# 2235854410/CCVPE

Hardware: AMD Instinct MI355X
Metric: query images/sec (VIGOR, 512x512 sat / 320x640 grd) (higher is better)
Workload: dtype f32; 1 GPU; vigor_samearea_fov360_b32; variant=vigor_ori_prior, batch_per_gpu=32, global_batch=32, parallelism=image-parallel x1, all_gather of 20 B/query results, schedule=two streams per GPU (aerial encoder + orientation decoder on the second)

## Files before the change

### ccvpe_amd/_lib.py

```python
from __future__ import annotations

import ctypes as C
import os

_HERE = os.path.dirname(os.path.abspath(__file__))
LIB_PATH = os.path.join(_HERE, "csrc", "libccvpe_hip.so")

OK = 0
VARIANT_ID = {"vigor": 0, "vigor_ori_prior": 1, "kitti": 2, "oxford": 3}


class Config(C.Structure):
    _fields_ = [("variant", C.c_int32), ("circular_padding", C.c_int32), ("ori_noise", C.c_float),
                ("device", C.c_int32), ("micro_batch", C.c_int32), ("reserved", C.c_int32 * 3)]


class Outputs(C.Structure):
    _fields_ = [("logits_flattened", C.c_void_p), ("heatmap", C.c_void_p), ("ori", C.c_void_p),
                ("matching_score", C.c_void_p * 6)]


class Pose(C.Structure):
    _fields_ = [("index", C.c_int32), ("prob", C.c_float), ("cos_v", C.c_float), ("sin_v", C.c_float),
                ("angle_deg", C.c_float)]
# ... 125 lines not shown
    ("ccvpe_localize_credible", C.c_int, [C.c_void_p, C.c_void_p, C.c_int32, C.c_int32, C.c_void_p, C.c_int32, C.c_void_p, C.c_int64,
                                          C.c_void_p, C.c_int32, C.c_void_p, C.c_void_p, C.c_void_p, C.c_void_p, C.c_void_p, C.c_void_p]),
    ("ccvpe_localize_credible_cached_indexed", C.c_int, [C.c_void_p, C.c_void_p, C.c_int32, C.c_int32, C.c_void_p, C.c_int32, C.c_void_p,
                                                         C.c_int32, C.c_void_p, C.c_int64, C.c_void_p, C.c_int32, C.c_void_p, C.c_void_p,
                                                         C.c_void_p, C.c_void_p, C.c_void_p, C.c_void_p]),
    ("ccvpe_preprocess",C.c_int, [C.c_void_p, C.c_int32, C.c_int32, C.c_int32, C.c_void_p, C.c_int32,
                                   C.POINTER(C.c_float * 3), C.POINTER(C.c_float * 3), C.c_void_p, C.c_void_p]),
    ("ccvpe_preprocess_resize", C.c_int, [C.c_void_p, C.c_int32, C.c_int32, C.c_int32, C.c_int32, C.c_int32, C.c_void_p, C.c_int32,
                                          C.POINTER(C.c_float * 3), C.POINTER(C.c_float * 3), C.c_void_p, C.c_void_p, C.c_void_p]),
    ("ccvpe_preprocess_affine", C.c_int, [C.c_void_p, C.c_int32, C.c_int32, C.c_int32, C.c_void_p, C.POINTER(C.c_int32), C.c_int32,
                                          C.c_int32, C.c_int32, C.c_int32, C.c_int32, C.POINTER(C.c_float * 3), C.POINTER(C.c_float * 3),
                                          C.c_void_p, C.c_void_p]),
    ("ccvpe_preprocess_window_resize", C.c_int, [C.c_void_p, C.c_int32, C.c_int32, C.c_void_p, C.c_int32, C.c_int32, C.c_int32,
                                                 C.c_int32, C.c_int32, C.POINTER(C.c_float * 3), C.POINTER(C.c_float * 3), C.c_void_p,
                                                 C.c_void_p, C.c_void_p]),
    ("ccvpe_set_debug", C.c_int, [C.c_void_p, C.c_int32]),
    ("ccvpe_set_streams", C.c_int, [C.c_void_p, C.c_int32]),
    ("ccvpe_read_tap", C.c_int, [C.c_void_p, C.c_char_p, C.c_void_p, C.c_size_t, C.POINTER(C.c_size_t),
                                 C.POINTER(C.c_int32 * 4)]),
    ("ccvpe_debug_dump_plan", C.c_int, [C.c_void_p, C.c_char_p]),
    ("ccvpe_profile_forward", C.c_int, [C.c_void_p, C.c_void_p, C.c_int32, C.c_int32, C.c_void_p, C.c_int32,
                                        C.POINTER(Outputs), C.c_void_p]),
    ("ccvpe_profile_row", C.c_int, [C.c_void_p, C.c_int32, C.c_char_p, C.c_size_t, C.POINTER(C.c_float),
                                    C.POINTER(C.c_double), C.POINTER(C.c_double)]),
    ("ccvpe_profile_row_issued", C.c_int, [C.c_void_p, C.c_int32, C.POINTER(C.c_double)]),
    ("ccvpe_op_num_tiles", C.c_int, []),
    ("ccvpe_op_tile_name", C.c_char_p, [C.c_int32]),
    ("ccvpe_op_conv2d", C.c_int, [C.c_void_p, C.c_int32, C.c_int32, C.c_int32, C.c_int32, C.c_void_p, C.c_void_p,
                                  C.c_int32, C.c_int32, C.c_int32, C.c_int32, C.c_int32, C.c_int32, C.c_int32,
                                  C.c_void_p, C.c_int32, C.POINTER(C.c_float), C.c_void_p]),
    ("ccvpe_op_conv2d_ex", C.c_int, [C.c_void_p, C.c_void_p]),
    ("ccvpe_op_level1", C.c_int, [C.c_void_p, C.c_int32, C.c_int32, C.c_int32, C.c_int32, C.c_int32, C.c_void_p, C.c_void_p,
                                  C.c_void_p, C.c_void_p, C.c_void_p, C.c_void_p, C.c_int32, C.c_int32, C.c_void_p, C.c_void_p]),
    ("ccvpe_op_pose_rows", C.c_int, [C.c_void_p, C.c_void_p, C.c_void_p, C.c_int32, C.c_void_p, C.c_void_p]),
]


IMAGENET_MEAN = (0.485, 0.456, 0.406)
IMAGENET_STD = (0.229, 0.224, 0.225)


def preprocess(img_u8_hwc, shift=None, crop_w=None, mean=IMAGENET_MEAN, std=IMAGENET_STD):
    import torch
    lib = load()
    assert img_u8_hwc.is_cuda and img_u8_hwc.dtype == torch.uint8 and img_u8_hwc.dim() == 4 and img_u8_hwc.shape[3] == 3
    img = img_u8_hwc.contiguous()
    B, H, W, _ = img.shape
    crop_w = W if crop_w is None else int(crop_w)
    out = torch.empty((B, 3, H, crop_w), dtype=torch.float32, device=img.device)
    sh = None
    if shift is not None:
        sh = torch.as_tensor(shift, dtype=torch.int32, device=img.device).contiguous()
        assert sh.numel() == B
    m = (C.c_float * 3)(*mean)
    s = (C.c_float * 3)(*std)
    stream = torch.cuda.current_stream(img.device).cuda_stream
    rc = lib.ccvpe_preprocess(C.c_void_p(img.data_ptr()), B, H, W, C.c_void_p(sh.data_ptr()) if sh is not None else None,
                              crop_w, C.byref(m), C.byref(s), C.c_void_p(out.data_ptr()), C.c_void_p(stream))
    check(rc, "ccvpe_preprocess")
    return out


def preprocess_resize(img_u8_hwc, out_hw, shift=None, crop_w=None, mean=IMAGENET_MEAN, std=IMAGENET_STD):
    import torch
    lib = load()
    assert img_u8_hwc.is_cuda and img_u8_hwc.dtype == torch.uint8 and img_u8_hwc.dim() == 4 and img_u8_hwc.shape[3] == 3
# ... 126 lines not shown
        assert resid.is_contiguous() and resid.dtype == torch.float32 and tuple(resid.shape[:3]) == (B, OH, OW)
        d.resid = resid.data_ptr(); d.resid_ld = resid.shape[3]
    assert 1 <= len(dsts) <= 3
    d.ndst = len(dsts)
    for i, (t, coff) in enumerate(dsts):
        assert t.is_cuda and t.is_contiguous() and t.dtype == torch.float32 and tuple(t.shape[:3]) == (B, OH, OW), tuple(t.shape)
        d.dst[i].ptr = t.data_ptr(); d.dst[i].ld = t.shape[3]; d.dst[i].coff = coff
    ran_tile, ran_split, runs = C.c_int32(0), C.c_int32(0), C.c_int32(-2)
    d.ran_tile, d.ran_split, d.requested_runs = C.pointer(ran_tile), C.pointer(ran_split), C.pointer(runs)
    stream = torch.cuda.current_stream(x.device).cuda_stream
    rc = lib.ccvpe_op_conv2d_ex(C.byref(d), C.c_void_p(stream))
    check(rc, "ccvpe_op_conv2d_ex")
    return [t for t, _ in dsts], lib.ccvpe_op_tile_name(ran_tile.value).decode(), ran_split.value, runs.value


def op_level1(x_nhwc, wd, bd, wa, ba, wt, bt, score=False, tile=1, max_wg=0):
    import torch
    lib = load()
    B, h, w, Cin = x_nhwc.shape
    Cout = wt.shape[0]
    x = x_nhwc.float()
    if score:
        x = torch.cat([x[..., :1], x.new_zeros((B, h, w, 7)), x[..., 1:]], dim=-1)
    x = x.contiguous()
    ws = [t.detach().float().contiguous() for t in (wd, bd, wa, ba, wt, bt)]
    out = torch.empty((B, Cout, 2 * h, 2 * w), dtype=torch.float32, device=x.device)
    stream = torch.cuda.current_stream(x.device).cuda_stream
    rc = lib.ccvpe_op_level1(C.c_void_p(x.data_ptr()), B, 2 * h, 2 * w, Cin, 1 if score else 0, *[C.c_void_p(t.data_ptr()) for t in ws],
                             Cout, tile | (max_wg << 8), C.c_void_p(out.data_ptr()), C.c_void_p(stream))
    check(rc, "ccvpe_op_level1")
    return out, rc


def op_pose_rows(handle, logits, ori):
    import torch
    lib = load()
    logits, ori = logits.detach().float().contiguous(), ori.detach().float().contiguous()
    B = logits.shape[0]
    rows = torch.empty((B, 5), dtype=torch.float32, device=logits.device)
    stream = torch.cuda.current_stream(logits.device).cuda_stream
    check(lib.ccvpe_op_pose_rows(handle, C.c_void_p(logits.data_ptr()), C.c_void_p(ori.data_ptr()), B, C.c_void_p(rows.data_ptr()),
                                 C.c_void_p(stream)), "ccvpe_op_pose_rows")
    return rows


_lib = None


def library_digest() -> str:
    override = os.environ.get("CCVPE_LIB_PATH")
    if override:
        import hashlib
        h = hashlib.sha256()
        with open(override, "rb") as fh:
            for chunk in iter(lambda: fh.read(1 << 20), b""):
                h.update(chunk)
        return h.hexdigest()
    from . import build as _build
    return _build._digest()


def load() -> C.CDLL:
    global _lib
    if _lib is not None:
        return _lib
    try:
# ... 42 lines not shown
```

### ccvpe_amd/build.py

```python
from __future__ import annotations

import hashlib
import os
import subprocess
import sys

HERE = os.path.dirname(os.path.abspath(__file__))
CSRC = os.path.join(HERE, "csrc")
LIB = os.path.join(CSRC, "libccvpe_hip.so")
STAMP = os.path.join(CSRC, ".libccvpe_hip.stamp")
SOURCES = ["ccvpe_api.hip", "ccvpe_weights.hip", "ccvpe_plan.hip", "ccvpe_tune.hip", "kernels_igemm.hip", "kernels_igemm_bf16x3.hip", "kernels_wino.hip", "kernels_wino4.hip", "kernels_wino4x.hip", "kernels_encoder.hip", "kernels_match.hip", "kernels_tail.hip", "kernels_heading.hip", "kernels_hprior.hip", "kernels_credible.hip", "kernels_track.hip", "kernels_track_affine.hip", "kernels_track_smooth.hip", "kernels_track_smooth_affine.hip", "kernels_track_link.hip", "kernels_track_viterbi.hip", "kernels_track_viterbi_affine.hip", "kernels_track_joint.hip", "kernels_track_joint_smooth.hip", "kernels_level1.hip", "kernels_level6.hip", "kernels_mbconv.hip", "kernels_preproc.hip", "kernels_warp.hip", "kernels_pw.hip", "kernels_proj.hip", "kernels_mbimg.hip"]
HEADERS = ["kernels.h", "ticket.h", "tail_shared.h", "track_blur.h", "track_maxmul.h", "track_smooth_work.h", "igemm_common.h", "ccvpe_internal.h", "kernels_level1_tile.inc", os.path.join("..", "..", "include", "ccvpe.h")]
FLAGS = ["--offload-arch=gfx950", "-O3", "-std=c++17", "-fPIC", "-ffp-contract=off", "-Wall", "-Wno-unused-function"]
EXTRA_FLAGS = {"kernels_match.hip": ["-fno-slp-vectorize"], "kernels_track.hip": ["-fno-slp-vectorize"], "kernels_track_affine.hip": ["-fno-slp-vectorize"],
               "kernels_track_smooth.hip": ["-fno-slp-vectorize"], "kernels_track_smooth_affine.hip": ["-fno-slp-vectorize"],
               "kernels_track_link.hip": ["-fno-slp-vectorize"],
               "kernels_track_viterbi.hip": ["-fno-slp-vectorize"], "kernels_track_viterbi_affine.hip": ["-fno-slp-vectorize"],
               "kernels_track_joint.hip": ["-fno-slp-vectorize"], "kernels_track_joint_smooth.hip": ["-fno-slp-vectorize"],
               "kernels_wino4.hip": ["-fno-slp-vectorize"], "kernels_wino4x.hip": ["-fno-slp-vectorize"], "kernels_level6.hip": ["-fno-slp-vectorize"]}


def _hipcc() -> str:
    for c in (os.environ.get("HIPCC"), "/opt/rocm/bin/hipcc", "hipcc"):
        if c and (os.path.isabs(c) and os.path.exists(c) or not os.path.isabs(c)):
            return c
    return "hipcc"


def _digest() -> str:
    h = hashlib.sha256()
    for f in SOURCES + HEADERS:
        with open(os.path.join(CSRC, f), "rb") as fh:
            h.update(fh.read())
    h.update(" ".join(FLAGS).encode())
    h.update(repr(sorted(EXTRA_FLAGS.items())).encode())
    return h.hexdigest()


def is_current() -> bool:
    if not (os.path.exists(LIB) and os.path.exists(STAMP)):
        return False
    with open(STAMP) as fh:
        return fh.read().strip() == _digest()

# ... 48 lines not shown
```

### ccvpe_amd/csrc/ccvpe_api.hip

```cpp
#include "ccvpe_internal.h"

namespace ccvpe { thread_local unsigned long long g_launches = 0; }
static thread_local std::string g_err_storage;
std::string& ccvpe_err() { return g_err_storage; }
int ccvpe_fail(int code, const char* fmt, ...) {
    char buf[1024];
    va_list ap;
    va_start(ap, fmt);
    vsnprintf(buf, sizeof(buf), fmt, ap);
    va_end(ap);
    g_err_storage = buf;
    return code;
}

__global__ __launch_bounds__(256) void checksum_kernel(const uint32_t* __restrict__ p, size_t n, unsigned long long* out) {
    unsigned long long s = 0;
    for (size_t i = (size_t)blockIdx.x * 256 + threadIdx.x; i < n; i += (size_t)gridDim.x * 256) s += (unsigned long long)p[i] * (unsigned long long)((i & 1023) + 1);
    for (int o = 32; o > 0; o >>= 1) s += __shfl_down(s, o);
    if ((threadIdx.x & 63) == 0) atomicAdd(out, s);
}


Switches read_switches() {
    Switches s;
    auto set = [](const char* name) { return getenv(name) != nullptr; };
    auto off = [](const char* name) { const char* e = getenv(name); return e && std::atoi(e) == 0; };
    if (const char* e = getenv("CCVPE_AUTOTUNE")) s.autotune = std::atoi(e) != 0;
    if (const char* e = getenv("CCVPE_FUSE_MBCONV")) s.fuse_mbconv = std::atoi(e);
    if (const char* e = getenv("CCVPE_FUSE_L1")) s.fuse_level1 = std::atoi(e) != 0;
    if (const char* e = getenv("CCVPE_L1_TILE")) s.l1_tile = std::atoi(e);
    if (const char* e = getenv("CCVPE_COMPOSE_L6")) s.compose_l6 = std::atoi(e);
    if (const char* e = getenv("CCVPE_SPLIT_L6")) s.split_l6 = std::atoi(e);
    if (const char* e = getenv("CCVPE_WINOGRAD")) s.wino = std::atoi(e) != 0;
    if (const char* e = getenv("CCVPE_GRAPH")) s.graph_mode = std::atoi(e) != 0;
    if (const char* e = getenv("CCVPE_STREAMS")) s.two_streams = std::atoi(e) >= 2;
    if (const char* e = getenv("CCVPE_PRECISION")) s.precision = (std::string(e) == "bf16x3") ? 1 : 0;
    s.stem_dw = !off("CCVPE_STEM_DW");
    if (const char* e = getenv("CCVPE_FRONT_SPREAD")) s.front_spread = std::atoi(e);
    s.mbconv_image = !off("CCVPE_MBCONV_IMAGE");
    s.se_ticket = !off("CCVPE_SE_TICKET");
    if (const char* e = getenv("CCVPE_SE_PROLOGUE")) s.se_prologue = std::atoi(e) == 1;
    s.split_planes = !set("CCVPE_NO_SPLIT_PLANES");
    s.match_prep_early = !off("CCVPE_MATCH_PREP_EARLY");
    s.match_wide = !off("CCVPE_MATCH_WIDE");
    s.issue_interleaved = !off("CCVPE_ISSUE_ORDER");
    s.log_schedule = set("CCVPE_LOG_SCHEDULE");
    s.no_reuse = set("CCVPE_NO_REUSE");
    s.tune_prefer_pw = set("CCVPE_TUNE_PREFER_PW");
    if (const char* e = getenv("CCVPE_TUNE_PREFER_PROJ")) { s.tune_prefer_proj = true; s.tune_prefer_lat = std::strcmp(e, "lat") == 0; }
    if (const char* e = getenv("CCVPE_TUNE_SPLITK")) s.tune_splitk = std::atoi(e);
    s.tune_no_bf16x3 = set("CCVPE_TUNE_NO_BF16X3");
    s.no_pw = set("CCVPE_NO_PW");
    s.tune_ignore_table = set("CCVPE_TUNE_IGNORE_TABLE");
    s.tune_lat_rows = set("CCVPE_TUNE_LAT_ROWS");
    s.tune_lat_split = set("CCVPE_TUNE_LAT_SPLIT");
    s.tune_no_fused_split = set("CCVPE_TUNE_NO_FUSED_SPLIT");
    if (const char* e = getenv("CCVPE_TUNE_VERBOSE")) s.tune_verbose = e;
    s.no_proj = set("CCVPE_NO_PROJ");
    if (const char* e = getenv("CCVPE_WINO4_MIN_N")) s.wino4_min_n = std::atoi(e);
    s.no_wino4 = set("CCVPE_NO_WINO4");
    s.no_wino4x = set("CCVPE_NO_WINO4X");
    s.pad_concat = !off("CCVPE_PAD_CONCAT");
    if (const char* e = getenv("CCVPE_DIAG_SYNC_BEFORE")) s.diag_sync = e;
    if (const char* e = getenv("CCVPE_DIAG_SNAP")) s.diag_snap = e;
    return s;
// ... 1765 lines not shown
int ccvpe_op_level1(const float* in, int32_t B, int32_t H, int32_t W, int32_t Cin, int32_t score, const float* wd, const float* bd,
                    const float* wa, const float* ba, const float* wt, const float* bt, int32_t Cout, int32_t tile, float* out, void* stream) {
    if (!in || !wd || !bd || !wa || !ba || !wt || !bt || !out) return ccvpe_fail(CCVPE_EINVAL, "null argument");
    const int cd = Cin - (score ? 1 : 0);
    if (B <= 0 || H <= 0 || W <= 0 || H % 16 || W % 16 || (Cout != 1 && Cout != 2) || cd <= 0 || cd % 4 || tile < 0 || (tile & 0xff) > 1 || ((tile >> 8) != 0 && (tile >> 8) < 8))
        return ccvpe_fail(CCVPE_EINVAL, "bad level-1 geometry (H, W multiples of 16, Cout 1 or 2, descriptor channels a multiple of 4, tile 0 or 1, workgroup cap 0 or >= 8)");
    if ((double)B * H * W * 16 >= 2147483647.0) return ccvpe_fail(CCVPE_EINVAL, "tensor exceeds 2^31 elements");
    std::vector<float> hwd((size_t)Cin * 64), hbd(16), hwa(16 * 16 * 9), hba(16), hwt((size_t)Cout * 16 * 9), hbt(Cout);
    HIPCHK(hipMemcpy(hwd.data(), wd, hwd.size() * sizeof(float), hipMemcpyDefault));
    HIPCHK(hipMemcpy(hbd.data(), bd, hbd.size() * sizeof(float), hipMemcpyDefault));
    HIPCHK(hipMemcpy(hwa.data(), wa, hwa.size() * sizeof(float), hipMemcpyDefault));
    HIPCHK(hipMemcpy(hba.data(), ba, hba.size() * sizeof(float), hipMemcpyDefault));
    HIPCHK(hipMemcpy(hwt.data(), wt, hwt.size() * sizeof(float), hipMemcpyDefault));
    HIPCHK(hipMemcpy(hbt.data(), bt, hbt.size() * sizeof(float), hipMemcpyDefault));
    ccvpe_handle_s tmp;
    DecoderW d;
    auto cleanup = [&]() { for (void* p : tmp.dev_allocs) (void)hipFree(p); };
    int rc = compose_level1(&tmp, d, hwd, hbd, hwa, hba, Cin, score ? 1 : 0);
    if (!rc) rc = pack_level1_tail(&tmp, d, hwt, hbt, Cout);
    if (rc) { cleanup(); return rc; }
    if (!level1_supported(d.l1_cxp)) { cleanup(); return ccvpe_fail(CCVPE_EINVAL, "the fused level takes up to 64 input channels"); }
    Level1Params lp = level1_params(d, d.l1_cx, B, Cout, Cout == 2);
    lp.x = in; lp.H = H; lp.W = W; lp.out = out; lp.raw = nullptr; lp.tile = tile & 0xff; lp.max_wg = tile >> 8;
    hipStream_t st = (hipStream_t)stream;
    launch_level1(lp, st);
    hipError_t e = hipGetLastError();
    hipError_t e2 = hipStreamSynchronize(st);
    cleanup();
    if (e != hipSuccess) return ccvpe_fail(CCVPE_EHIP, "level-1 launch failed: %s", hipGetErrorString(e));
    if (e2 != hipSuccess) return ccvpe_fail(CCVPE_EHIP, "level-1 execution failed: %s", hipGetErrorString(e2));
    return level1_tile(lp);
}

}
```

### ccvpe_amd/csrc/ccvpe_internal.h

```cpp
#pragma once
#include "../../include/ccvpe.h"
#include "kernels.h"

#include <algorithm>
#include <cmath>
#include <cstdarg>
#include <cstdio>
#include <cstdlib>
#include <cstring>
#include <functional>
#include <map>
#include <memory>
#include <optional>
#include <set>
#include <string>
#include <type_traits>
#include <vector>

using namespace ccvpe;

std::string& ccvpe_err();
int ccvpe_fail(int code, const char* fmt, ...);
#define HIPCHK(expr)                                                                           \
    do {                                                                                       \
// ... 46 lines not shown
        for (int i = 0; i < 6; ++i) {
            s.match_ch[i] = mc[i]; s.step[i] = st[i];
            s.head_ch[i] = (v == CCVPE_VARIANT_OXFORD) ? ho[i] : hv[i];
        }
        s.feat_h = (v == CCVPE_VARIANT_OXFORD) ? 4 : 10;
        s.sat_desc = 1280; s.n_rolls = 20; s.centre = (v == CCVPE_VARIANT_OXFORD);
        cp(s.loc, VIGOR_LOC); cp(s.ori, VIGOR_ORI);
    }
    return s;
}

static void static_pad(int k, int s, int& lo, int& hi) {
    if (s == 1) { lo = hi = (k - 1) / 2; return; }
    int total = k - 2;
    lo = total / 2; hi = total - lo;
}
static int conv_out(int n, int k, int s) {
    int lo, hi; static_pad(k, s, lo, hi);
    return (n + lo + hi - k) / s + 1;
}
static int se_squeeze(int cin) { return std::max(1, (int)(cin * 0.25)); }
static int round_up(int a, int b) { return (a + b - 1) / b * b; }
static int deconv_width(const DecLevel& l, bool pad) {
    return (pad && l.skip > 0 && (l.dout * 4) % 64 != 0) ? round_up(l.dout, 16) : l.dout;
}

struct Switches {
    bool autotune = true;
    int fuse_mbconv = 1;
    bool fuse_level1 = true;
    int l1_tile = 1;
    std::optional<int> compose_l6;
    std::optional<int> split_l6;
    bool wino = true;
    int graph_mode = 0;
    bool two_streams = true;
    std::optional<int> precision;
    bool stem_dw = true;
    std::optional<int> front_spread;
    bool mbconv_image = true;
    bool se_ticket = true;
    bool se_prologue = false;
    bool split_planes = true;
    bool match_prep_early = true;
    bool match_wide = true;
    bool issue_interleaved = true;
    bool log_schedule = false;
    bool no_reuse = false;
    bool tune_prefer_pw = false;
    bool tune_prefer_proj = false;
    bool tune_prefer_lat = false;
    std::optional<int> tune_splitk;
    bool tune_no_bf16x3 = false;
    bool no_pw = false;
    bool tune_ignore_table = false;
    bool tune_lat_rows = false;
    bool tune_lat_split = false;
    bool tune_no_fused_split = false;
    std::string tune_verbose;
    bool no_proj = false;
    int wino4_min_n = 40;
    bool no_wino4 = false;
    bool no_wino4x = false;
    bool pad_concat = true;
    std::string diag_sync, diag_snap;

// ... 30 lines not shown
    size_t proj_bytes = 0;
};
struct BlockW {
    PackedConv expand, project;
    float* exp_lin = nullptr;
    int exp_cinp = 0;
    float *dw_w = nullptr, *dw_b = nullptr, *se_w1 = nullptr, *se_b1 = nullptr, *se_w2 = nullptr, *se_b2 = nullptr;
    int sq = 0;
};
struct EncoderW {
    float *stem_w = nullptr, *stem_b = nullptr;
    BlockW blk[16];
    PackedConv head;
};
struct DecoderW {
    PackedConv deconv[6], conva[6], convb[5];
    float* tail_w = nullptr;
    float* l1_wt = nullptr;
    float tail_b[2] = {0.f, 0.f};
    float *l1_wc = nullptr, *l1_ws = nullptr, *l1_bc = nullptr;
    int l1_cx = 0, l1_cxp = 0, l1_c0 = 0, l1_ng = 0, l1_score = 0;
};
struct Level6W {
    float* wc = nullptr;
    float* bc = nullptr;
    PackedConv skip;
    int K = 0, Kc = 0, N = 0, Npad = 0;
    float* wb = nullptr;
    float* ws = nullptr;
};
static constexpr int LEVEL6_AUTO_MIN_BATCH = 8;
static constexpr int LEVEL6_SPLIT_MIN_BATCH = 8;
enum { SPLIT6_CONV_B = 1, SPLIT6_SKIP = 2 };
struct ccvpe_handle_s;
struct DecoderW;
int level6_shape(const ccvpe_handle_s* h, const DecoderW& d, const struct DecLevel& l, int& K, int& Kc, int& N, int& Npad);
int ensure_level6(ccvpe_handle_s* h, int wm);
int ensure_level6_split(ccvpe_handle_s* h);
void release_level6(ccvpe_handle_s* h);
int compose_level1(ccvpe_handle_s* h, DecoderW& d, const std::vector<float>& w, const std::vector<float>& b, const std::vector<float>& wa,
                   const std::vector<float>& ba, int cin, int nscore);
int pack_level1_tail(ccvpe_handle_s* h, DecoderW& d, const std::vector<float>& w2, const std::vector<float>& b2, int cout);

struct Tensor {
    int id = -1; int B = 0, H = 0, W = 0, C = 0;
    bool split = false;
    long long numel() const { return (long long)B * H * W * C; }
};

struct TailCall {
    float* rows = nullptr;
    int topk_k = 0, topk_r = 0;
    const float* log_prior = nullptr;
    long long prior_stride = 0;
    float* stats = nullptr;
    float* posterior = nullptr;
    float* summary = nullptr;
    int summary_r = 0;
    float* heading = nullptr;
    float* hist = nullptr;
    int heading_bins = 0, heading_r = 0;
    const float* hprior_table = nullptr;
    int hprior_stride = 0, hprior_nb = 0;
    float* cred = nullptr;
    int cred_levels = 0;
    float cred_level[CRED_MAX_LEVELS] = {0.f, 0.f, 0.f, 0.f, 0.f, 0.f, 0.f, 0.f};
// ... 357 lines not shown
```

### ccvpe_amd/csrc/ccvpe_plan.hip

```cpp
#include "ccvpe_internal.h"

static int window_offset(const VariantSpec& vs, int level, int L) {
    const int C = vs.match_ch[level];
    return vs.centre ? (int)((double)C / 2 - (double)L / 2) : 0;
}
static int mod(int a, int m) { int r = a % m; return r < 0 ? r + m : r; }

ConvParams conv_params(const PackedConv& pc, const float* in, int in_ld, int B, int H, int W, int OH, int OW,
                              int stride, int pad_t, int pad_l, int act) {
    ConvParams p{};
    p.in = in; p.in_ld = in_ld; p.B = B; p.H = H; p.W = W; p.Cin = pc.cinp; p.OH = OH; p.OW = OW;
    p.KH = pc.KH; p.KW = pc.KW; p.stride = stride; p.pad_t = pad_t; p.pad_l = pad_l;
    p.wpk = pc.w; p.w_hi = pc.w_hi; p.w_lo = pc.w_lo; p.Kpad = pc.Kpad; p.Npad = round_up(pc.N, conv_igemm_npad()); p.nchunks = pc.nchunks; p.bias = pc.bias; p.N = pc.N; p.act = act;
    p.gate = nullptr; p.resid = nullptr; p.resid_ld = 0; p.ndst = 0; p.mode = MODE_CONV; p.deconv_cout = 0;
    p.M = B * OH * OW;
    p.in_bytes = (unsigned)((size_t)B * H * W * in_ld * sizeof(float));
    p.gate_bytes = (unsigned)((size_t)B * pc.cinp * sizeof(float));
    p.w_plane_bytes = (unsigned)((size_t)p.Npad * pc.Kpad * sizeof(unsigned short));
    p.wino_w = pc.wino; p.wino_n16 = pc.wino_n16; p.wino_bytes = (unsigned)pc.wino_bytes;
    p.wino4_w = pc.wino4; p.wino4_bytes = (unsigned)pc.wino4_bytes;
    p.wino4x_w = pc.wino4x; p.wino4x_bytes = (unsigned)pc.wino4x_bytes; p.wino4x_cfg = pc.wino4x_cfg;
    p.proj_w = pc.proj; p.proj_bytes = (unsigned)pc.proj_bytes;
    return p;
}
// ... 386 lines not shown
    const int hout = 16;
    const Level6W* w6 = &h->l6[&dw == &h->ori ? 1 : 0];
    const Level6Params lp = l6.p[&dw == &h->ori ? 1 : 0];
    const int G = 4 * level6_positions(l6.wm);
    Tensor V = pl.alloc(G, 1, lp.R, lp.Kc), Mp = pl.alloc(G, 1, lp.R, lp.N), sk = pl.alloc(B, hout, hout, l.mid);
    const Tensor s15 = l6.skip15;
    pl.add(tag + ".l6_transform", {din, V}, [=](const Ctx& c) {
        Level6Params q = lp; q.x = c.ptr(din); q.v = c.ptr(V);
        launch_level6_transform(q, c.stream);
    }, 0.0, 4.0 * ((double)din.numel() + (double)V.numel()));
    pl.add(tag + ".l6_gemm", {V, Mp}, [=](const Ctx& c) {
        Level6Params q = lp; q.v = c.ptr(V); q.wc = w6->wc; q.mp = c.ptr(Mp);
        launch_level6_gemm(q, c.stream);
    }, 2.0 * G * lp.R * (double)lp.N * lp.Kc, 4.0 * ((double)V.numel() + (double)G * lp.Npad * lp.Kc + (double)Mp.numel()));
    if (l6.split & SPLIT6_SKIP) {
        Split6Params sp = l6.ss[&dw == &h->ori ? 1 : 0];
        sp.x_ld = s15.C;
        plan_split6(pl, sp, &w6->ws, nullptr, false, s15, sk, tag, "skip");
    } else {
        const PackedConv* pc = &w6->skip;
        pl.add_conv(tag + ".conv_skip", {s15, sk}, B * hout * hout, lp.N, round_up(9 * l.skip, 32), [=](const Ctx& c, int tile) {
            ConvParams p = conv_params(*pc, c.ptr(s15), s15.C, B, hout, hout, hout, hout, 1, 1, 1, ACT_NONE);
            p.dst[0] = c.dst(sk); p.ndst = 1;
            c.launch_conv(p, tile);
        }, 2.0 * B * hout * hout * 9.0 * s15.C * l.mid, 4.0 * B * hout * hout * ((double)s15.C + l.mid));
        set_skip6_flags(h, pl.ops.back(), s15.C, l.skip, lp.N);
    }
    pl.add(tag + ".l6_combine", {Mp, sk, mid}, [=](const Ctx& c) {
        Level6Params q = lp; q.mp = c.ptr(Mp); q.skip = c.ptr(sk); q.bc = w6->bc; q.out = c.ptr(mid);
        launch_level6_combine(q, c.stream);
    }, 0.0, 4.0 * ((double)Mp.numel() + 2.0 * (double)mid.numel()));
}

static Tensor plan_level(ccvpe_handle_s* h, Plan& pl, int B, const Level6Form& l6, const DecoderW& dw, const DecLevel* lv, int j, Tensor din, Tensor cat,
                         const std::string& tag) {
    const int hin = 8 << j, hout = hin * 2;
    const DecLevel& l = lv[j];
    Tensor mid = pl.alloc(B, hout, hout, l.mid);
    if (j == 0 && l6.wm) {
        plan_level6_composed(h, pl, B, l6, dw, l, din, mid, tag);
    } else {
        {
            const PackedConv* pc = &dw.deconv[j];
            const int cout = deconv_width(l, h->sw.pad_concat);
            pl.add_conv(tag + ".deconv", {din, cat}, B * hin * hin, pc->N, pc->Kpad, [=](const Ctx& c, int tile) {
                ConvParams p = conv_params(*pc, c.ptr(din), din.C, B, hin, hin, hin, hin, 1, 0, 0, ACT_NONE);
                p.mode = MODE_DECONV; p.deconv_cout = cout;
                p.dst[0] = c.dst(cat); p.ndst = 1;
                c.launch_conv(p, tile);
            }, 2.0 * B * hin * hin * (double)l.din * 4 * l.dout, 4.0 * B * hin * hin * ((double)din.C + 4.0 * l.dout));
            pl.ops.back().is_pw = !din.split;
            pl.ops.back().proj_ok = pc->proj != nullptr && !din.split && h->cfg.reserved[0] == 0;
        }
        mid.split = cat.split;
        const PackedConv* pc = &dw.conva[j];
        pl.add_conv(tag + ".conv_a", {cat, mid}, B * hout * hout, pc->N, pc->Kpad, [=](const Ctx& c, int tile) {
            ConvParams p = conv_params(*pc, c.ptr(cat), cat.C, B, hout, hout, hout, hout, 1, 1, 1, ACT_RELU);
            p.in_split = cat.split; p.in_plane_bytes = (unsigned)(cat.numel() * 2);
            p.dst[0] = c.dst(mid); p.ndst = 1;
            c.launch_conv(p, tile);
        }, 2.0 * B * hout * hout * 9.0 * cat.C * l.mid, 4.0 * B * hout * hout * ((double)cat.C + l.mid));
        set_conv3x3_flags(h, pl.ops.back(), *pc, cat);
    }
    if (j == 5) return mid;
    Tensor o = pl.alloc(B, hout, hout, l.out);
    const PackedConv* pc = &dw.convb[j];
    if (j == 0 && l6.wm && (l6.split & SPLIT6_CONV_B)) {
        const int d = &dw == &h->ori ? 1 : 0;
        plan_split6(pl, l6.sb[d], &h->l6[d].wb, &pc->bias, false, mid, o, tag, "b");
        return o;
    }
    pl.add_conv(tag + ".conv_b", {mid, o}, B * hout * hout, pc->N, pc->Kpad, [=](const Ctx& c, int tile) {
        ConvParams p = conv_params(*pc, c.ptr(mid), mid.C, B, hout, hout, hout, hout, 1, 1, 1, ACT_NONE);
        p.in_split = mid.split; p.in_plane_bytes = (unsigned)(mid.numel() * 2);
        p.dst[0] = {c.ptr(o), o.C, 0}; p.ndst = 1;
// ... 488 lines not shown
```

### ccvpe_amd/csrc/kernels.h

```cpp
#pragma once
#include <functional>
#include <vector>
#include <hip/hip_runtime.h>
#include <stdint.h>
#include "ticket.h"

namespace ccvpe {

extern thread_local unsigned long long g_launches;
#define CCVPE_LAUNCH(...) do { ++::ccvpe::g_launches; hipLaunchKernelGGL(__VA_ARGS__); } while (0)

struct LdsAttr { size_t set[16] = {0}; };
inline void ensure_dynamic_lds(LdsAttr& state, const void* kernel, size_t bytes) {
    int dev = 0;
    if (hipGetDevice(&dev) != hipSuccess || dev < 0 || dev >= 16) dev = 0;
    if (bytes > state.set[dev] && hipFuncSetAttribute(kernel, hipFuncAttributeMaxDynamicSharedMemorySize, (int)bytes) == hipSuccess) state.set[dev] = bytes;
}

enum Act { ACT_NONE = 0, ACT_RELU = 1, ACT_SWISH = 2 };

struct Dst {
    float* ptr;
    int ld;
    int coff;
// ... 291 lines not shown
struct Level6ComposeParams {
    int wm;
    const float* dw;
    int cw, dout, dkpad;
    const float* aw;
    int cinw, akpad;
    int K, Kc, N, Npad;
    double* w2;
    float* wc;
};
void launch_level6_compose(const Level6ComposeParams& p, hipStream_t s);

struct Split6Params {
    int B, C, Kc;
    int N, Npad;
    int R, bm;
    const float* x;
    int x_ld, x_coff;
    float* v;
    const float* wc;
    float* mp;
    const float* bias;
    int relu;
    float* out;
    int out_ld, out_coff;
};
int split6_rows(int B, int* bm_out);
bool split6_supported(const Split6Params& p);
Level6Params split6_gemm_params(const Split6Params& p);
void launch_split6_transform(const Split6Params& p, hipStream_t s);
void launch_split6_inverse(const Split6Params& p, hipStream_t s);
void conv_wino4_filter(const double g[3][3], double u[36]);

__device__ __forceinline__ float pose_angle_deg(float cs, float sn) {
    float ang = acosf(fminf(fmaxf(cs, -1.f), 1.f)) * 57.29577951308232f;
    if (sn < 0.f) { ang = fmodf(-ang, 360.f); if (ang < 0.f) ang += 360.f; }
    return ang;
}

static constexpr int TAIL_HW = 512, TAIL_CHUNKS = 64;
static_assert(TAIL_HW * TAIL_HW == TAIL_CHUNKS * 4 * 4 * 256 && TAIL_CHUNKS == 64, "four float4 per thread per chunk, one lane of a wave per chunk");

struct SoftmaxParams {
    const float* logits;
    int B, n;
    float* partial;
    int chunks;
    float* out;
    const float* prior;
    long long prior_stride;
};
void launch_softmax(const SoftmaxParams& p, hipStream_t s);
void launch_softmax_partial(const SoftmaxParams& p, hipStream_t s);

struct PoseArgmaxParams {
    const float* logits;
    const float* partial;
    int B, n, chunks;
    float* pairs;
    unsigned* tickets;
    int* index;
    float* rows;
    float* stats;
    const float* prior;
    long long prior_stride;
    float* posterior;
// ... 387 lines not shown
```

### include/ccvpe.h

```cpp
#ifndef CCVPE_H
#define CCVPE_H

#include <stddef.h>
#include <stdint.h>

#ifdef __cplusplus
extern "C" {
#endif

#define CCVPE_OK 0
#define CCVPE_EINVAL (-1)
#define CCVPE_ESTATE (-2)
#define CCVPE_EHIP (-3)
#define CCVPE_ENOMEM (-4)
#define CCVPE_EKEY (-5)

#define CCVPE_VARIANT_VIGOR 0
#define CCVPE_VARIANT_VIGOR_ORI_PRIOR 1
#define CCVPE_VARIANT_KITTI 2
#define CCVPE_VARIANT_OXFORD 3

#define CCVPE_OUT_HW 512
#define CCVPE_SAT_HW 512

// ... 254 lines not shown
int ccvpe_profile_row(ccvpe_handle h, int32_t i, char* name_buf, size_t name_cap, float* ms,
                      double* flops, double* bytes);
int ccvpe_profile_row_issued(ccvpe_handle h, int32_t i, double* issued_flops);

int ccvpe_op_num_tiles(void);
const char* ccvpe_op_tile_name(int32_t tile);
int ccvpe_op_conv2d(const float* in, int32_t B, int32_t H, int32_t W, int32_t Cin, const float* w, const float* bias,
                    int32_t Cout, int32_t KH, int32_t KW, int32_t stride, int32_t pad, int32_t act, int32_t tile,
                    float* out, int32_t iters, float* ms, void* stream);

enum { CCVPE_OP_CONV = 0, CCVPE_OP_DECONV = 1 };
typedef struct ccvpe_op_conv_dst { float* ptr; int32_t ld, coff; } ccvpe_op_conv_dst;
typedef struct ccvpe_op_conv_desc {
    const float* in;
    int32_t B, H, W, Cin, in_ld;
    const float* w;
    const float* bias;
    int32_t Cout, KH, KW, stride, pad, act, tile, mode;
    const float* gate;
    const float* resid;
    int32_t resid_ld, ndst;
    ccvpe_op_conv_dst dst[3];
    int32_t iters;
    float* ms;
    int32_t* ran_tile;
    int32_t* ran_split;
    int32_t* requested_runs;
} ccvpe_op_conv_desc;
int ccvpe_op_conv2d_ex(const ccvpe_op_conv_desc* d, void* stream);

int ccvpe_op_level1(const float* in, int32_t B, int32_t H, int32_t W, int32_t Cin, int32_t score, const float* wd, const float* bd,
                    const float* wa, const float* ba, const float* wt, const float* bt, int32_t Cout, int32_t tile, float* out, void* stream);

int ccvpe_op_pose_rows(ccvpe_handle h, const float* logits, const float* ori, int32_t batch, float* rows, void* stream);

#ifdef __cplusplus
}
#endif
#endif
```

Baseline: 2763 queries/s.

## Add dedicated MFMA kernel for 2x2 stride-2 transposed convs in decoder

Adds a specialised kernel for the decoder's k2s2 transposed convolutions. It computes all four taps in one pass with f32 MFMA from LDS-resident weights, skips dead (zero-padded score) input channels, and scatters the results straight into the strided concat buffer. It replaces the generic packed pointwise conv path at decoder levels 3-4 when the batch is large enough, and is selectable through an environment switch. The aim is less redundant input reading and less generic igemm overhead. The cost is a new code path with fixed shape constraints and possible LDS and occupancy limits.

```diff
diff --git a/ccvpe_amd/_lib.py b/ccvpe_amd/_lib.py
--- a/ccvpe_amd/_lib.py
+++ b/ccvpe_amd/_lib.py
@@ -181,6 +181,8 @@
     ("ccvpe_op_conv2d_ex", C.c_int, [C.c_void_p, C.c_void_p]),
     ("ccvpe_op_level1", C.c_int, [C.c_void_p, C.c_int32, C.c_int32, C.c_int32, C.c_int32, C.c_int32, C.c_void_p, C.c_void_p,
                                   C.c_void_p, C.c_void_p, C.c_void_p, C.c_void_p, C.c_int32, C.c_int32, C.c_void_p, C.c_void_p]),
+    ("ccvpe_op_deconv_k2s2", C.c_int, [C.c_void_p, C.c_int32, C.c_int32, C.c_int32, C.c_int32, C.c_int32, C.c_void_p, C.c_void_p, C.c_int32,
+                                       C.c_void_p, C.c_int32, C.c_int32, C.c_int32, C.c_void_p]),
     ("ccvpe_op_pose_rows", C.c_int, [C.c_void_p, C.c_void_p, C.c_void_p, C.c_int32, C.c_void_p, C.c_void_p]),
 ]
 
@@ -373,6 +375,23 @@
     return out, rc
 
 
+def op_deconv_k2s2(x_nhwc, w, bias, dst, coff=0, cw=None):
+    import torch
+    lib = load()
+    x = x_nhwc.contiguous()
+    B, H, W, in_ld = x.shape
+    w = w.detach().float().contiguous()
+    Cin, Cout = w.shape[0], w.shape[1]
+    b = bias.detach().float().contiguous() if bias is not None else None
+    assert dst.is_cuda and dst.is_contiguous() and dst.dtype == torch.float32 and tuple(dst.shape[:3]) == (B, 2 * H, 2 * W), tuple(dst.shape)
+    stream = torch.cuda.current_stream(x.device).cuda_stream
+    rc = lib.ccvpe_op_deconv_k2s2(C.c_void_p(x.data_ptr()), B, H, W, Cin, in_ld, C.c_void_p(w.data_ptr()),
+                                  C.c_void_p(b.data_ptr()) if b is not None else None, Cout, C.c_void_p(dst.data_ptr()), dst.shape[3], coff,
+                                  Cout if cw is None else cw, C.c_void_p(stream))
+    check(rc, "ccvpe_op_deconv_k2s2")
+    return rc
+
+
 def op_pose_rows(handle, logits, ori):
     import torch
     lib = load()
diff --git a/ccvpe_amd/build.py b/ccvpe_amd/build.py
--- a/ccvpe_amd/build.py
+++ b/ccvpe_amd/build.py
@@ -9,7 +9,7 @@
 CSRC = os.path.join(HERE, "csrc")
 LIB = os.path.join(CSRC, "libccvpe_hip.so")
 STAMP = os.path.join(CSRC, ".libccvpe_hip.stamp")
-SOURCES = ["ccvpe_api.hip", "ccvpe_weights.hip", "ccvpe_plan.hip", "ccvpe_tune.hip", "kernels_igemm.hip", "kernels_igemm_bf16x3.hip", "kernels_wino.hip", "kernels_wino4.hip", "kernels_wino4x.hip", "kernels_encoder.hip", "kernels_match.hip", "kernels_tail.hip", "kernels_heading.hip", "kernels_hprior.hip", "kernels_credible.hip", "kernels_track.hip", "kernels_track_affine.hip", "kernels_track_smooth.hip", "kernels_track_smooth_affine.hip", "kernels_track_link.hip", "kernels_track_viterbi.hip", "kernels_track_viterbi_affine.hip", "kernels_track_joint.hip", "kernels_track_joint_smooth.hip", "kernels_level1.hip", "kernels_level6.hip", "kernels_mbconv.hip", "kernels_preproc.hip", "kernels_warp.hip", "kernels_pw.hip", "kernels_proj.hip", "kernels_mbimg.hip"]
+SOURCES = ["ccvpe_api.hip", "ccvpe_weights.hip", "ccvpe_plan.hip", "ccvpe_tune.hip", "kernels_igemm.hip", "kernels_igemm_bf16x3.hip", "kernels_wino.hip", "kernels_wino4.hip", "kernels_wino4x.hip", "kernels_encoder.hip", "kernels_match.hip", "kernels_tail.hip", "kernels_heading.hip", "kernels_hprior.hip", "kernels_credible.hip", "kernels_track.hip", "kernels_track_affine.hip", "kernels_track_smooth.hip", "kernels_track_smooth_affine.hip", "kernels_track_link.hip", "kernels_track_viterbi.hip", "kernels_track_viterbi_affine.hip", "kernels_track_joint.hip", "kernels_track_joint_smooth.hip", "kernels_level1.hip", "kernels_level6.hip", "kernels_mbconv.hip", "kernels_preproc.hip", "kernels_warp.hip", "kernels_pw.hip", "kernels_deconv.hip", "kernels_proj.hip", "kernels_mbimg.hip"]
 HEADERS = ["kernels.h", "ticket.h", "tail_shared.h", "track_blur.h", "track_maxmul.h", "track_smooth_work.h", "igemm_common.h", "ccvpe_internal.h", "kernels_level1_tile.inc", os.path.join("..", "..", "include", "ccvpe.h")]
 FLAGS = ["--offload-arch=gfx950", "-O3", "-std=c++17", "-fPIC", "-ffp-contract=off", "-Wall", "-Wno-unused-function"]
 EXTRA_FLAGS = {"kernels_match.hip": ["-fno-slp-vectorize"], "kernels_track.hip": ["-fno-slp-vectorize"], "kernels_track_affine.hip": ["-fno-slp-vectorize"],
diff --git a/ccvpe_amd/csrc/ccvpe_api.hip b/ccvpe_amd/csrc/ccvpe_api.hip
--- a/ccvpe_amd/csrc/ccvpe_api.hip
+++ b/ccvpe_amd/csrc/ccvpe_api.hip
@@ -31,6 +31,7 @@
     if (const char* e = getenv("CCVPE_L1_TILE")) s.l1_tile = std::atoi(e);
     if (const char* e = getenv("CCVPE_COMPOSE_L6")) s.compose_l6 = std::atoi(e);
     if (const char* e = getenv("CCVPE_SPLIT_L6")) s.split_l6 = std::atoi(e);
+    if (const char* e = getenv("CCVPE_DECONV_K2S2")) s.deconv_k2s2 = std::atoi(e);
     if (const char* e = getenv("CCVPE_WINOGRAD")) s.wino = std::atoi(e) != 0;
     if (const char* e = getenv("CCVPE_GRAPH")) s.graph_mode = std::atoi(e) != 0;
     if (const char* e = getenv("CCVPE_STREAMS")) s.two_streams = std::atoi(e) >= 2;
@@ -1862,4 +1863,42 @@
     return level1_tile(lp);
 }
 
-}
+int ccvpe_op_deconv_k2s2(const float* in, int32_t B, int32_t H, int32_t W, int32_t Cin, int32_t in_ld, const float* w, const float* bias, int32_t Cout,
+                         float* out, int32_t ld, int32_t coff, int32_t cw, void* stream) {
+    if (!in || !w || !out) return ccvpe_fail(CCVPE_EINVAL, "null argument");
+    if (B <= 0 || H <= 0 || W <= 0 || Cin <= 0 || Cin % 8 || Cout <= 0 || cw < Cout || in_ld < Cin)
+        return ccvpe_fail(CCVPE_EINVAL, "bad transposed-conv geometry (Cin a multiple of 8, in_ld >= Cin, cw >= Cout)");
+    std::vector<float> hw((size_t)Cin * Cout * 4), b1(Cout, 0.f), hb(4 * (size_t)cw, 0.f);
+    HIPCHK(hipMemcpy(hw.data(), w, hw.size() * sizeof(float), hipMemcpyDefault));
+    if (bias) HIPCHK(hipMemcpy(b1.data(), bias, Cout * sizeof(float), hipMemcpyDefault));
+    for (int q = 0; q < 4; ++q) std::copy(b1.begin(), b1.end(), hb.begin() + (size_t)q * cw);
+    std::vector<unsigned char> live(Cin, 0);
+    for (int c = 0; c < Cin; ++c)
+        for (int i = 0; i < Cout * 4 && !live[c]; ++i) live[c] = hw[(size_t)c * Cout * 4 + i] != 0.f;
+    DeconvK2S2Params kp{};
+    kp.B = B; kp.H = H; kp.W = W; kp.Cin = Cin; kp.in_ld = in_ld; kp.Kpad = round_up(Cin, 32);
+    kp.ld = ld; kp.coff = coff; kp.cw = cw;
+    if (!deconv_k2s2_prepare(kp, live.data()))
+        return ccvpe_fail(CCVPE_EINVAL, "deconv_k2s2_kernel does not take these sizes (cw a multiple of 16 up to 80, in_ld, ld and coff multiples of 4, coff + cw <= ld, "
+                                        "at most 192 live input channels, weights of two taps within the LDS)");
+    ccvpe_handle_s tmp;
+    tmp.sw = read_switches();
+    PackedConv pc;
+    int rc = pack_conv(&tmp, pc, 4 * cw, 1, Cin, Cin, identity_map(Cin),
+                       [&](int n, int, int c) { const int q = n / cw, o = n % cw; return o < Cout ? hw[((size_t)c * Cout + o) * 4 + q] : 0.f; }, hb, 1, 1);
+    auto cleanup = [&]() { for (void* p : tmp.dev_allocs) (void)hipFree(p); };
+    if (rc) { cleanup(); return rc; }
+    if (pc.Kpad < Cin || pc.N != 4 * cw) { cleanup(); return ccvpe_fail(CCVPE_ESTATE, "unexpected packed form"); }
+    kp.Kpad = pc.Kpad;
+    kp.x = in; kp.wpk = pc.w; kp.bias = pc.bias; kp.out = out;
+    hipStream_t st = (hipStream_t)stream;
+    launch_deconv_k2s2(kp, st);
+    hipError_t e = hipGetLastError();
+    hipError_t e2 = hipStreamSynchronize(st);
+    cleanup();
+    if (e != hipSuccess) return ccvpe_fail(CCVPE_EHIP, "transposed-conv launch failed: %s", hipGetErrorString(e));
+    if (e2 != hipSuccess) return ccvpe_fail(CCVPE_EHIP, "transposed-conv execution failed: %s", hipGetErrorString(e2));
+    return kp.taps;
+}
+
+}
diff --git a/ccvpe_amd/csrc/ccvpe_internal.h b/ccvpe_amd/csrc/ccvpe_internal.h
--- a/ccvpe_amd/csrc/ccvpe_internal.h
+++ b/ccvpe_amd/csrc/ccvpe_internal.h
@@ -102,6 +102,7 @@
     int l1_tile = 1;
     std::optional<int> compose_l6;
     std::optional<int> split_l6;
+    std::optional<int> deconv_k2s2;
     bool wino = true;
     int graph_mode = 0;
     bool two_streams = true;
@@ -198,6 +199,8 @@
 static constexpr int LEVEL6_AUTO_MIN_BATCH = 8;
 static constexpr int LEVEL6_SPLIT_MIN_BATCH = 8;
 enum { SPLIT6_CONV_B = 1, SPLIT6_SKIP = 2 };
+static constexpr int DECONV_K2S2_MIN_BATCH = 8;
+static constexpr int DECONV_K2S2_MIN_BATCH_L3 = 16;
 struct ccvpe_handle_s;
 struct DecoderW;
 int level6_shape(const ccvpe_handle_s* h, const DecoderW& d, const struct DecLevel& l, int& K, int& Kc, int& N, int& Npad);
diff --git a/ccvpe_amd/csrc/ccvpe_plan.hip b/ccvpe_amd/csrc/ccvpe_plan.hip
--- a/ccvpe_amd/csrc/ccvpe_plan.hip
+++ b/ccvpe_amd/csrc/ccvpe_plan.hip
@@ -442,6 +442,21 @@
     }, 0.0, 4.0 * ((double)Mp.numel() + 2.0 * (double)mid.numel()));
 }
 
+static bool deconv_k2s2_planned(const ccvpe_handle_s* h, int B, int j, const PackedConv& pc, const DecLevel& l, const Tensor& din, const Tensor& cat, int cw,
+                                DeconvK2S2Params& kp) {
+    if (h->cfg.reserved[0] != 0 || din.split || cat.split || j < 2 || j > 4) return false;
+    const int sw = h->sw.deconv_k2s2 ? *h->sw.deconv_k2s2 : -1;
+    if (sw == 0 || (sw < 0 && (j < 3 || B < (j == 3 ? DECONV_K2S2_MIN_BATCH_L3 : DECONV_K2S2_MIN_BATCH)))) return false;
+    if (pc.N != 4 * cw || pc.cinp <= 0 || pc.cinp > din.C || pc.KH != 1 || pc.KW != 1) return false;
+    std::vector<unsigned char> live(pc.cinp, 1);
+    if (pc.cinp == l.din + score_pad(1) - 1) { for (int c = 1; c < score_pad(1); ++c) live[c] = 0; }
+    else if (pc.cinp != l.din) return false;
+    const int hin = 8 << j;
+    kp.B = B; kp.H = hin; kp.W = hin; kp.Cin = pc.cinp; kp.in_ld = din.C; kp.Kpad = pc.Kpad;
+    kp.ld = cat.C; kp.coff = 0; kp.cw = cw;
+    return deconv_k2s2_prepare(kp, live.data());
+}
+
 static Tensor plan_level(ccvpe_handle_s* h, Plan& pl, int B, const Level6Form& l6, const DecoderW& dw, const DecLevel* lv, int j, Tensor din, Tensor cat,
                          const std::string& tag) {
     const int hin = 8 << j, hout = hin * 2;
@@ -450,7 +465,18 @@
     if (j == 0 && l6.wm) {
         plan_level6_composed(h, pl, B, l6, dw, l, din, mid, tag);
     } else {
-        {
+        const PackedConv* pcd = &dw.deconv[j];
+        const int cwd = deconv_width(l, h->sw.pad_concat);
+        DeconvK2S2Params kp{};
+        const double dflops = 2.0 * B * hin * hin * (double)l.din * 4 * l.dout, dbytes = 4.0 * B * hin * hin * ((double)din.C + 4.0 * l.dout);
+        if (deconv_k2s2_planned(h, B, j, *pcd, l, din, cat, cwd, kp)) {
+            pl.add(tag + ".deconv", {din, cat}, [=](const Ctx& c) {
+                DeconvK2S2Params q = kp;
+                q.x = c.ptr(din); q.wpk = pcd->w; q.bias = pcd->bias; q.out = c.ptr(cat);
+                launch_deconv_k2s2(q, c.stream);
+            }, dflops, dbytes);
+            pl.ops.back().form = "conv_pw_k2s2";
+        } else {
             const PackedConv* pc = &dw.deconv[j];
             const int cout = deconv_width(l, h->sw.pad_concat);
             pl.add_conv(tag + ".deconv", {din, cat}, B * hin * hin, pc->N, pc->Kpad, [=](const Ctx& c, int tile) {
diff --git a/ccvpe_amd/csrc/kernels.h b/ccvpe_amd/csrc/kernels.h
--- a/ccvpe_amd/csrc/kernels.h
+++ b/ccvpe_amd/csrc/kernels.h
@@ -347,6 +347,25 @@
 void launch_split6_inverse(const Split6Params& p, hipStream_t s);
 void conv_wino4_filter(const double g[3][3], double u[36]);
 
+struct DeconvK2S2Params {
+    static constexpr int MAX_GROUPS = 48;
+    const float* x;
+    int B, H, W, Cin, in_ld;
+    const float* wpk;
+    int Kpad;
+    const float* bias;
+    float* out;
+    int ld, coff, cw;
+    int ngroups;
+    unsigned jmasked;
+    unsigned short gch[MAX_GROUPS];
+    unsigned char gmask[MAX_GROUPS];
+    int taps;
+    unsigned fdw_mul, fdw_shift, fdh_mul, fdh_shift;
+};
+bool deconv_k2s2_prepare(DeconvK2S2Params& p, const unsigned char* live);
+void launch_deconv_k2s2(const DeconvK2S2Params& p, hipStream_t s);
+
 __device__ __forceinline__ float pose_angle_deg(float cs, float sn) {
     float ang = acosf(fminf(fmaxf(cs, -1.f), 1.f)) * 57.29577951308232f;
     if (sn < 0.f) { ang = fmodf(-ang, 360.f); if (ang < 0.f) ang += 360.f; }
diff --git a/ccvpe_amd/csrc/kernels_deconv.hip b/ccvpe_amd/csrc/kernels_deconv.hip
--- /dev/null
+++ b/ccvpe_amd/csrc/kernels_deconv.hip
@@ -0,0 +1,219 @@
+#include "igemm_common.h"
+
+#include <algorithm>
+
+namespace ccvpe {
+
+static constexpr int DK_WAVES = 8;
+static constexpr size_t DK_LDS_MAX = 160 * 1024;
+
+static size_t deconv_k2s2_lds(int taps, int cw, int J) {
+    return ((size_t)taps * cw * (16 * J + 4) + (size_t)taps * cw + (size_t)DK_WAVES * 16 * (cw + 4) + DK_WAVES * 16 + DeconvK2S2Params::MAX_GROUPS) * sizeof(float);
+}
+
+template <int JMAX, int CT, int TAPS>
+__global__ __launch_bounds__(64 * DK_WAVES, (JMAX == 6 && CT <= 3 && CT * TAPS <= 8) ? 4 : 2) void deconv_k2s2_kernel(const DeconvK2S2Params p) {
+    constexpr int CW = 16 * CT, NT = CT * TAPS, LDC = CW + 4, C4 = CW / 4;
+    extern __shared__ __attribute__((aligned(16))) float smem[];
+    const int J = p.ngroups >> 2;
+    const int ldb = 16 * J + 4;
+    float* Bs = smem;
+    float* bias_s = Bs + NT * 16 * ldb;
+    float* Cs = bias_s + NT * 16;
+    int* rowb = reinterpret_cast<int*>(Cs + DK_WAVES * 16 * LDC);
+    int* gtab = rowb + DK_WAVES * 16;
+
+    const int tid = threadIdx.x, lane = tid & 63, wave = tid >> 6;
+    const int q0 = TAPS == 2 ? 2 * (int)blockIdx.y : 0;
+    const int M = p.B * p.H * p.W;
+
+    if (tid < p.ngroups) gtab[tid] = ((int)p.gch[tid] << 4) | (int)p.gmask[tid];
+    if (tid < NT * 16) bias_s[tid] = p.bias[q0 * CW + tid];
+    {
+        const int g4 = p.ngroups;
+        for (int i = tid; i < NT * 16 * g4; i += 64 * DK_WAVES) {
+            const int n = i / g4, g = i - n * g4;
+            const int c = p.gch[g], mk = p.gmask[g];
+            f32x4 w = *reinterpret_cast<const f32x4*>(p.wpk + (size_t)(q0 * CW + n) * p.Kpad + c);
+#pragma unroll
+            for (int e = 0; e < 4; ++e) w[e] = (mk >> e) & 1 ? w[e] : 0.f;
+            *reinterpret_cast<f32x4*>(Bs + n * ldb + g * 4) = w;
+        }
+    }
+    __syncthreads();
+
+    const int mtiles = (M + 15) >> 4;
+    const int kq = lane >> 4, kq4 = 4 * kq;
+    const int wg = xcd_remap(blockIdx.x, gridDim.x);
+    int mt = wg * DK_WAVES + wave;
+    const int mt_stride = gridDim.x * DK_WAVES;
+    if (mt >= mtiles) return;
+
+    int gt[JMAX];
+#pragma unroll
+    for (int j = 0; j < JMAX; ++j) gt[j] = j < J ? gtab[j * 4 + kq] : 0;
+
+    float* cw = Cs + wave * 16 * LDC;
+    int* rb = rowb + wave * 16;
+    const float* bp = Bs + (lane & 15) * ldb + kq4;
+
+    f32x4 acur[JMAX], anext[JMAX];
+    auto load_tile = [&](int mtile, f32x4* dst) {
+        const int m = min(mtile * 16 + (lane & 15), M - 1);
+        const float* row = p.x + (size_t)m * p.in_ld;
+#pragma unroll
+        for (int j = 0; j < JMAX; ++j)
+            if (j < J) dst[j] = *reinterpret_cast<const f32x4*>(row + (gt[j] >> 4));
+    };
+    load_tile(mt, acur);
+
+    const int ow_ld = 2 * p.W * p.ld;
+    f32x4 acc[NT];
+    while (mt < mtiles) {
+        load_tile(mt + mt_stride, anext);
+        {
+            const int m = mt * 16 + (lane & 15);
+            const int t = fast_div(m, p.fdw_mul, p.fdw_shift);
+            const int x = m - t * p.W;
+            const int b = fast_div(t, p.fdh_mul, p.fdh_shift);
+            const int y = t - b * p.H;
+            const int o = ((b * 2 * p.H + 2 * y) * 2 * p.W + 2 * x) * p.ld + p.coff;
+            if (lane < 16) rb[lane] = m < M ? o : -1;
+        }
+#pragma unroll
+        for (int t = 0; t < NT; ++t) acc[t] = f32x4{0.f, 0.f, 0.f, 0.f};
+        __builtin_amdgcn_sched_barrier(0);
+#pragma unroll
+        for (int j = 0; j < JMAX; ++j) {
+            if (j < J) {
+                f32x4 a = acur[j];
+                if ((p.jmasked >> j) & 1) {
+#pragma unroll
+                    for (int e = 0; e < 4; ++e) a[e] = (gt[j] >> e) & 1 ? a[e] : 0.f;
+                }
+                static_assert(NT % 2 == 0, "column tiles are taken in pairs");
+#pragma unroll
+                for (int t = 0; t < NT; t += 2) {
+                    const f32x4 b0 = *reinterpret_cast<const f32x4*>(bp + t * 16 * ldb + j * 16);
+                    const f32x4 b1 = *reinterpret_cast<const f32x4*>(bp + (t + 1) * 16 * ldb + j * 16);
+                    acc[t] = __builtin_amdgcn_mfma_f32_16x16x4f32(b0.x, a.x, acc[t], 0, 0, 0);
+                    acc[t + 1] = __builtin_amdgcn_mfma_f32_16x16x4f32(b1.x, a.x, acc[t + 1], 0, 0, 0);
+                    acc[t] = __builtin_amdgcn_mfma_f32_16x16x4f32(b0.y, a.y, acc[t], 0, 0, 0);
+                    acc[t + 1] = __builtin_amdgcn_mfma_f32_16x16x4f32(b1.y, a.y, acc[t + 1], 0, 0, 0);
+                    acc[t] = __builtin_amdgcn_mfma_f32_16x16x4f32(b0.z, a.z, acc[t], 0, 0, 0);
+                    acc[t + 1] = __builtin_amdgcn_mfma_f32_16x16x4f32(b1.z, a.z, acc[t + 1], 0, 0, 0);
+                    acc[t] = __builtin_amdgcn_mfma_f32_16x16x4f32(b0.w, a.w, acc[t], 0, 0, 0);
+                    acc[t + 1] = __builtin_amdgcn_mfma_f32_16x16x4f32(b1.w, a.w, acc[t + 1], 0, 0, 0);
+                }
+            }
+        }
+        __builtin_amdgcn_sched_barrier(0);
+#pragma unroll
+        for (int q = 0; q < TAPS; ++q) {
+#pragma unroll
+            for (int t = 0; t < CT; ++t) {
+                const f32x4 bv = *reinterpret_cast<const f32x4*>(bias_s + (q * CT + t) * 16 + kq4);
+                *reinterpret_cast<f32x4*>(cw + (lane & 15) * LDC + t * 16 + kq4) = acc[q * CT + t] + bv;
+            }
+            __builtin_amdgcn_s_waitcnt(0xC07F);
+            __builtin_amdgcn_wave_barrier();
+            const int toff = ((q0 + q) >> 1) * ow_ld + ((q0 + q) & 1) * p.ld;
+#pragma unroll
+            for (int r = 0; r < CT; ++r) {
+                const int it = lane + 64 * r;
+                const int row = it / C4, c4 = it - row * C4;
+                const int o = rb[row];
+                const f32x4 v = *reinterpret_cast<const f32x4*>(cw + row * LDC + c4 * 4);
+                if (o >= 0) *reinterpret_cast<f32x4*>(p.out + (size_t)(unsigned)(o + toff + c4 * 4)) = v;
+                __builtin_amdgcn_sched_barrier(0);
+                asm volatile("s_nop 1");
+                __builtin_amdgcn_sched_barrier(0);
+            }
+            __builtin_amdgcn_s_waitcnt(0xC07F);
+            __builtin_amdgcn_wave_barrier();
+        }
+#pragma unroll
+        for (int j = 0; j < JMAX; ++j) acur[j] = anext[j];
+        mt += mt_stride;
+    }
+}
+
+static void make_fast_div(unsigned d, unsigned& mul, unsigned& shift) {
+    unsigned l = 0;
+    while ((1u << l) < d) ++l;
+    mul = (unsigned)((((unsigned long long)1 << 32) * (((unsigned long long)1 << l) - d)) / d + 1);
+    shift = l;
+}
+
+bool deconv_k2s2_prepare(DeconvK2S2Params& p, const unsigned char* live) {
+    if (p.B <= 0 || p.H <= 0 || p.W <= 0 || p.Cin <= 0 || p.Cin % 4 || p.in_ld < p.Cin || p.in_ld % 4 || p.Kpad < p.Cin || p.Kpad % 4) return false;
+    if (p.cw <= 0 || p.cw % 16 || p.cw > 80 || p.ld % 4 || p.coff % 4 || p.coff < 0 || p.coff + p.cw > p.ld) return false;
+    if ((double)p.B * p.H * p.W * p.in_ld >= 2147483647.0 || 4.0 * p.B * p.H * p.W * p.ld >= 2147483647.0) return false;
+    int n = 0;
+    unsigned jm = 0;
+    for (int c = 0; c < p.Cin; c += 4) {
+        int mk = 0;
+        for (int e = 0; e < 4; ++e) mk |= (!live || live[c + e]) ? 1 << e : 0;
+        if (!mk) continue;
+        if (n == DeconvK2S2Params::MAX_GROUPS) return false;
+        p.gch[n] = (unsigned short)c; p.gmask[n] = (unsigned char)mk;
+        if (mk != 15) jm |= 1u << (n >> 2);
+        ++n;
+    }
+    if (n == 0) { p.gch[0] = 0; p.gmask[0] = 0; jm |= 1u; n = 1; }
+    while (n % 4) {
+        p.gch[n] = 0; p.gmask[n] = 0; jm |= 1u << (n >> 2); ++n;
+    }
+    p.ngroups = n; p.jmasked = jm;
+    const int J = n / 4, ct = p.cw / 16;
+    if (ct <= 4 && deconv_k2s2_lds(4, p.cw, J) <= DK_LDS_MAX) p.taps = 4;
+    else if (ct >= 3 && deconv_k2s2_lds(2, p.cw, J) <= DK_LDS_MAX) p.taps = 2;
+    else return false;
+    make_fast_div((unsigned)p.W, p.fdw_mul, p.fdw_shift);
+    make_fast_div((unsigned)p.H, p.fdh_mul, p.fdh_shift);
+    return true;
+}
+
+template <int JMAX, int CT, int TAPS>
+static void launch_dk(const DeconvK2S2Params& p, hipStream_t s) {
+    const size_t lds = deconv_k2s2_lds(TAPS, p.cw, p.ngroups / 4);
+    static LdsAttr attr;
+    auto kern = deconv_k2s2_kernel<JMAX, CT, TAPS>;
+    ensure_dynamic_lds(attr, reinterpret_cast<const void*>(kern), lds);
+    const int mtiles = (p.B * p.H * p.W + 15) / 16;
+    const int ny = 4 / TAPS;
+    static size_t occ_lds[16] = {0};
+    static int occ[16] = {0};
+    int dev = 0;
+    if (hipGetDevice(&dev) != hipSuccess || dev < 0 || dev >= 16) dev = 0;
+    if (occ_lds[dev] != lds) {
+        int n = 0;
+        if (hipOccupancyMaxActiveBlocksPerMultiprocessor(&n, kern, 64 * DK_WAVES, lds) != hipSuccess) { (void)hipGetLastError(); n = 1; }
+        occ[dev] = std::max(1, std::min(2, n)); occ_lds[dev] = lds;
+    }
+    const int per_cu = occ[dev];
+    const int gx = std::max(1, std::min((mtiles + DK_WAVES - 1) / DK_WAVES, 256 * per_cu / ny));
+    CCVPE_LAUNCH(kern, dim3(gx, ny), dim3(64 * DK_WAVES), lds, s, p);
+}
+
+template <int JMAX>
+static void launch_dk_j(const DeconvK2S2Params& p, hipStream_t s) {
+    const int ct = p.cw / 16;
+    if (p.taps == 4) {
+        if (ct == 1) launch_dk<JMAX, 1, 4>(p, s);
+        else if (ct == 2) launch_dk<JMAX, 2, 4>(p, s);
+        else if (ct == 3) launch_dk<JMAX, 3, 4>(p, s);
+        else launch_dk<JMAX, 4, 4>(p, s);
+    } else {
+        if (ct == 3) launch_dk<JMAX, 3, 2>(p, s);
+        else if (ct == 4) launch_dk<JMAX, 4, 2>(p, s);
+        else launch_dk<JMAX, 5, 2>(p, s);
+    }
+}
+
+void launch_deconv_k2s2(const DeconvK2S2Params& p, hipStream_t s) {
+    if (p.ngroups <= 24) launch_dk_j<6>(p, s);
+    else launch_dk_j<12>(p, s);
+}
+
+}
diff --git a/include/ccvpe.h b/include/ccvpe.h
--- a/include/ccvpe.h
+++ b/include/ccvpe.h
@@ -310,6 +310,9 @@
 int ccvpe_op_level1(const float* in, int32_t B, int32_t H, int32_t W, int32_t Cin, int32_t score, const float* wd, const float* bd,
                     const float* wa, const float* ba, const float* wt, const float* bt, int32_t Cout, int32_t tile, float* out, void* stream);
 
+int ccvpe_op_deconv_k2s2(const float* in, int32_t B, int32_t H, int32_t W, int32_t Cin, int32_t in_ld, const float* w, const float* bias, int32_t Cout,
+                         float* out, int32_t ld, int32_t coff, int32_t cw, void* stream);
+
 int ccvpe_op_pose_rows(ccvpe_handle h, const float* logits, const float* ori, int32_t batch, float* rows, void* stream);
 
 #ifdef __cplusplus
```

Result: faster. 2797 queries/s, median of 6 (+1.3%).
